# limacv/VideoLoop3D

Measured on AMD Instinct MI355X. Metric: rendered Mpix/s (fwd+bwd) D=32 planes 720p, higher is better.
Workload: dtype f32; 1 GPU; cfg3 stage-2 MPV render fwd+bwd: D=32 planes, T=50 frames, 720x1280, mpv convention, plane stack (D,T,H,W,4) f32 resident in HBM; parallelism=single GPU, variant=0

## Files before the change

videoloop3d_amd/csrc/vl3d_render_bwd_choice.h:

```cpp
#pragma once
#include <stdint.h>
#include "vl3d.h"

namespace vl3d_render_detail {

enum BwdPolicy : int {
    BWD_NONE = 0,
    BWD_AUTO,
    BWD_TILE16,
    BWD_FLAT8,
    BWD_NARROW32,
    BWD_PAIRS32,
    BWD_PAIRS64X12,
};
struct BwdSetting {
    BwdPolicy policy;
    bool gather9;
    bool owner4;
};

inline BwdSetting bwd_setting_of(int entry, int bv, bool tile_ok, bool has_quad_map) {
    BwdSetting s{BWD_NONE, bv == 4, bv != 3 && bv != 4};
    if (entry == VL3D_BWD_ENTRY_ADAM) {
        s.gather9 = s.owner4 = false;
        s.policy = has_quad_map ? (bv == 3 ? BWD_TILE16 : BWD_NARROW32) : BWD_AUTO;
    } else if (bv == 1 || !tile_ok) {
        s.policy = BWD_NONE;
    } else if (entry == VL3D_BWD_ENTRY_MASK) {
        s.policy = (bv == 3 || bv == 4) ? BWD_TILE16 : BWD_FLAT8;
    } else {
        s.policy = bv == 0 ? BWD_AUTO : bv == 2 ? BWD_FLAT8 : bv == 5 ? BWD_NARROW32 : bv == 6 ? BWD_PAIRS32 : bv == 7 ? BWD_PAIRS64X12 : BWD_TILE16;
    }
    return s;
}

enum BwdShape : int { BWD_64X16 = 0, BWD_64X8, BWD_32X16, BWD_64X12, BWD_NSHAPES };
struct BwdRegion { int width, rows; };
constexpr BwdRegion BWD_REGIONS[BWD_NSHAPES] = {{64, 16}, {64, 8}, {32, 16}, {64, 12}};
constexpr int BWD_HALO = 1;
constexpr int bwd_interior_w(int shape) { return BWD_REGIONS[shape].width - 2 * BWD_HALO; }
constexpr int bwd_interior_h(int shape) { return BWD_REGIONS[shape].rows - 2 * BWD_HALO; }
constexpr int bwd_slot_bits(int shape) { return BWD_REGIONS[shape].width * BWD_REGIONS[shape].rows > 512 ? 10 : 9; }

constexpr BwdRegion BWD_SIZING_ONLY_INTERIORS[] = {{60, 12}, {28, 12}};
inline int64_t bwd_max_tiles(int H, int W) {
    auto ntiles = [&](int iw, int ih) { return (int64_t)((W + iw - 1) / iw) * ((H + ih - 1) / ih); };
    int64_t tiles = 0;
    for (int s = 0; s < BWD_NSHAPES; ++s) tiles = ntiles(bwd_interior_w(s), bwd_interior_h(s)) > tiles ? ntiles(bwd_interior_w(s), bwd_interior_h(s)) : tiles;
    for (const BwdRegion &r : BWD_SIZING_ONLY_INTERIORS) tiles = ntiles(r.width, r.rows) > tiles ? ntiles(r.width, r.rows) : tiles;
    return tiles;
}

struct BwdChoice {
    int family;
    BwdShape shape;
    bool reg, mask, adam, cull, f16;
    bool owner4;
};

constexpr int bwd_key(int family, int shape, bool reg, bool mask = false, bool adam = false) {
    return family | shape << 2 | (int)reg << 5 | (int)mask << 6 | (int)adam << 7;
}
inline int bwd_key(const BwdChoice &c) { return bwd_key(c.family, c.shape, c.reg, c.mask, c.adam); }

struct BwdFacts {
    int coord, border, order, ract, aact;
    bool f16;
    int plane_record;
    int T, H, W, Hs, Ws;
    BwdSetting set;
    bool reg, mask, adam, qk, gcu;
};

inline BwdChoice choose_bwd(const BwdFacts &f) {
    const BwdPolicy p = f.set.policy;
    const bool sig = f.ract == VL3D_ACT_SIGMOID && f.aact == VL3D_ACT_SIGMOID;
    const bool shipped = f.coord == VL3D_COORD_AFFINE && f.border == VL3D_BORDER_HARDCUT && f.order == VL3D_ACT_POST && sig && !f.f16;
    const bool shipped9 = shipped && f.plane_record == 9;
    BwdChoice c{VL3D_BWD_TILE, BWD_64X16, false, false, false, false, false, false};
    c.owner4 = f.T == 1 && !f.adam && f.set.owner4;
    if (p == BWD_NONE) { c.family = VL3D_BWD_ATOMICS; c.owner4 = false; return c; }
    if (f.mask && shipped) { c.shape = p == BWD_FLAT8 ? BWD_64X8 : BWD_64X16; c.reg = f.reg; c.mask = true; return c; }
    if (f.adam && shipped9) {
        c.adam = true;
        if (f.qk) { c.shape = p == BWD_TILE16 ? BWD_64X16 : BWD_32X16; c.reg = c.cull = true; return c; }
        c.family = VL3D_BWD_PAIR; c.shape = BWD_32X16; c.reg = f.reg;
        return c;
    }
    if (sig && f.T >= 2 && !f.qk) {
        const bool fits = (int64_t)f.Hs * 100 <= (int64_t)f.H * 107 || (int64_t)f.Ws * 100 <= (int64_t)f.W * 107;
        if ((p == BWD_AUTO || p == BWD_PAIRS32 || p == BWD_PAIRS64X12) && !f.reg && fits) {
            c.family = p == BWD_PAIRS32 ? VL3D_BWD_PAIR : VL3D_BWD_PAIR12;
            c.shape = p == BWD_PAIRS32 ? BWD_32X16 : BWD_64X12;
            c.f16 = f.f16;
            return c;
        }
        if (f.coord != VL3D_COORD_UTILS_MPI && p == BWD_AUTO && f.reg) {
            c.family = VL3D_BWD_PAIR; c.shape = BWD_32X16; c.reg = true; c.f16 = f.f16;
            return c;
        }
    }
    if (shipped9 && (p == BWD_NARROW32 || (p == BWD_AUTO && f.qk && f.gcu))) {
        c.shape = BWD_32X16; c.reg = f.reg || (p == BWD_NARROW32 && f.qk && f.gcu); c.cull = f.qk;
        return c;
    }
    if (shipped9 && !f.reg && !f.qk && (p == BWD_FLAT8 || (p == BWD_AUTO && f.T == 1))) { c.shape = BWD_64X8; return c; }
    c.reg = f.reg || (f.qk && f.gcu); c.cull = f.qk; c.f16 = f.f16;
    return c;
}

}
```

videoloop3d_amd/csrc/vl3d_render_core.h:

```cpp
#pragma once
#include <stddef.h>
#include "vl3d_common.h"
#include "vl3d_bake_rule.h"

#include "vl3d_adam.h"
#include "vl3d_render_bwd_choice.h"

#ifndef VL3D_HS
#define VL3D_HS 9
#define VL3D_HN 9
#endif

namespace vl3d_render_detail {

#ifndef VL3D_PAIR_MIN_WAVES
#define VL3D_PAIR_MIN_WAVES 4
#endif
#ifndef VL3D_FWD2X_MIN_WAVES
#define VL3D_FWD2X_MIN_WAVES 4
#endif

#ifdef VL3D_REG_ABLATE
#define VL3D_REGAB(bit) ((VL3D_REG_ABLATE & (bit)) != 0)
#else
// ... 1388 lines not shown
                }
            continue;
        }
        float2 tc = make_float2(0.f, 0.f);
        float4 gval = make_float4(0.f, 0.f, 0.f, 0.f);
        f4 o = f4{0.f, 0.f, 0.f, 0.f}, pre = o;
        Taps2 tp{};
        float gm = 0.f, msig = 0.f;
        if (inimg) {
            if constexpr (CULL) tp = make_taps2<COORD, BORDER>(h, px, py, a.Hs, a.Ws, a.sx, a.sy, a.ox, a.oy, plane_cull(a, d));
            else tp = make_taps2<COORD, BORDER>(h, px, py, a.Hs, a.Ws, a.sx, a.sy, a.ox, a.oy);
            const char *src = plane;
            if VL3D_ABLATE(a.ablate, 4) {
                src = reinterpret_cast<const char *>(a.stack);
                tp.off &= 0xfff0u;
            }
            typename TapVal<F16, ORDER>::type tv[4];
            load_taps2<F16>(src, tp, st, tv);
            float mt[4];
            if constexpr (MASK) load_mask_taps(mplane, tp.off, st, mt);
            o = shade2<ORDER, RACT, AACT>(tp, tv, &pre);
            if constexpr (MASK) msig = act_fwd<VL3D_ACT_SIGMOID>(mask_blend(mt, tp.w));
        }
        f4 sg = f4{0.f, 0.f, 0.f, 0.f};
        if constexpr (REG) if (reg_on) {
            if ((d >> 2) != wg_idx) {
                wg_idx = d >> 2;
                const uint2 *w = sgp + (size_t)(d >> 2) * sg_plane;
                const uint2 zz = make_uint2(0x55555555u, 0x55555555u);
                wg_own = w[0]; wg_l = w[has_l ? -1 : 0]; wg_u = w[has_u ? -(ptrdiff_t)a.W : 0];
                if (!has_l) wg_l = zz;
                if (!has_u) wg_u = zz;
                if (fl & 12u) wg_p = reinterpret_cast<const uint2 *>(a.reg_patch)[w - reinterpret_cast<const uint2 *>(a.reg_signs)];
            }
            const bool hi = (d & 2) != 0;
            sg = reg_grad32(hi ? wg_own.y : wg_own.x, hi ? wg_l.y : wg_l.x, hi ? wg_u.y : wg_u.x, hi ? wg_p.y : wg_p.x, 16u * (d & 1), fl,
                            f4{gsx_c, gsx_c, gsx_c, gsx_a}, f4{gsy_c, gsy_c, gsy_c, gsy_a});
        }
        if (inimg) {
            const float q = dot3p(Gr, o.x, Gg, o.y, Gb, o.z, gA);
            const float w = o.w * Tr;
            if constexpr (MASK) gm = gL * w * (msig * (1.0f - msig));
            P = fmaf(w, q, P);
            const float om = 1.0f - o.w;
            const float behind = (om > 1e-12f) ? (S - P) * fast_rcp(om) : 0.0f;
            if constexpr (REG) sg.w += fmaf(gN2, o.w, gN1);
            gval = make_float4(fmaf(w, Gr, sg.x), fmaf(w, Gg, sg.y), fmaf(w, Gb, sg.z), fmaf(Tr, q, -behind) + sg.w);
            Tr *= om;
            if constexpr (ORDER == VL3D_ACT_POST)
                gval = make_float4(gval.x * act_bwd<RACT>(pre.x, o.x), gval.y * act_bwd<RACT>(pre.y, o.y),
                                   gval.z * act_bwd<RACT>(pre.z, o.z), gval.w * act_bwd<AACT>(pre.w, o.w));
            tc = make_float2(tp.tx, tp.ty);
            if (!(tp.cov > 0.0f && provider)) gval = make_float4(0.f, 0.f, 0.f, 0.f);
        }
        s_t[buf][tid] = tc;
        s_g[buf][tid] = gval;
        if constexpr (MASK) s_gm[buf][tid] = gm;
        f4 pre_m = f4{0.f, 0.f, 0.f, 0.f}, pre_v = pre_m, pre_p = pre_m;
        if constexpr (ADAM && CULL) {
            const bool mine0 = row < wh && lane < ww && (e0 >> SLOT_BITS) == my_tile && (rec0.x & 3u) == 1u;
            const size_t fb = adam_frame_base(a, d, t), o = mine0 ? (size_t)rec0.y << 4 : 0;
            pre_m = *reinterpret_cast<const f4 *>(reinterpret_cast<const char *>(a.ad.m) + fb + o);
            pre_v = *reinterpret_cast<const f4 *>(reinterpret_cast<const char *>(a.ad.v) + fb + o);
            pre_p = load_texel<false>(plane, mine0 ? (win0 + toff_thread) << 4 : 0u);
            asm volatile("" ::: "memory");
        }
        __syncthreads();
        if VL3D_ABLATE(a.ablate, 1) continue;
        auto gather = [&](unsigned e, int wx, int wy, unsigned tix, uint2 rec = make_uint2(0u, 0u), bool pre = false) {
            if ((e >> SLOT_BITS) != my_tile) return;
            const int lc = (int)(e & SLOT_MASK);
            const f2 tau = f2{(float)(X0 + wx), (float)(Y0 + wy)};
            f4 acc = f4{0.f, 0.f, 0.f, 0.f};
            float accm = 0.f;
            if VL3D_ABLATE(a.ablate, 8) {
            } else if (apart) {
                const f2 c0 = *reinterpret_cast<const f2 *>(&s_t[buf][lc]);
                const int li0 = lc - (tau.x < c0.x ? 1 : 0) - (tau.y < c0.y ? RW : 0);
#pragma unroll
                for (int k = 0; k < 4; ++k) {
                    const int li = li0 + (k >> 1) * RW + (k & 1);
                    const f2 dc = *reinterpret_cast<const f2 *>(&s_t[buf][li]) - tau;
                    const float wgt = tent_weight(dc.x) * tent_weight(dc.y);
                    acc += *reinterpret_cast<const f4 *>(&s_g[buf][li]) * wgt;
                    if constexpr (MASK) accm = fmaf(s_gm[buf][li], wgt, accm);
                }
            } else {
#pragma unroll
            for (int dy = -1; dy <= 1; ++dy)
#pragma unroll
                for (int dx = -1; dx <= 1; ++dx) {
                    const int li = lc + dy * RW + dx;
                    const f2 dc = *reinterpret_cast<const f2 *>(&s_t[buf][li]) - tau;
                    const float wgt = tent_weight(dc.x) * tent_weight(dc.y);
                    if (!a.gather9 && __builtin_amdgcn_ballot_w64(wgt != 0.0f) == 0ull) continue;
                    acc += *reinterpret_cast<const f4 *>(&s_g[buf][li]) * wgt;
                    if constexpr (MASK) accm = fmaf(s_gm[buf][li], wgt, accm);
                }
            }
            if constexpr (ORDER == VL3D_ACT_PRE || ORDER == VL3D_ACT_BAKED) {
                const f4 sv = load_texel<F16>(plane, tix << 4);
                acc = f4{acc.x * act_bwd<RACT>(sv.x, act_fwd<RACT>(sv.x)), acc.y * act_bwd<RACT>(sv.y, act_fwd<RACT>(sv.y)),
                         acc.z * act_bwd<RACT>(sv.z, act_fwd<RACT>(sv.z)), acc.w * act_bwd<AACT>(sv.w, act_fwd<AACT>(sv.w))};
            }
            if constexpr (ADAM) {
                int from;
                if constexpr (CULL) {
                    const unsigned c = rec.x & 3u;
                    if (c == 2) store_grad_texel<false>(gplane, tix << 4, acc);
                    if (c != 1) return;
                    from = (int)(rec.x >> 2);
                    const size_t offp = (size_t)rec.y << 4;
                    if (pre) adam_texel_step_mv(a, adam_frame_base(a, d, t), offp, from, pre_p, acc, pre_m, pre_v);
                    else adam_texel_step(a, adam_frame_base(a, d, t), offp, from, load_texel<false>(plane, tix << 4), acc);
                } else {
                    unsigned off;
                    if (!adam_texel(a, d, X0 + wx, Y0 + wy, from, off)) return;
                    adam_texel_step(a, adam_frame_base(a, d, t), off, from, load_texel<false>(plane, tix << 4), acc);
                }
            } else if (!VL3D_ABLATE(a.ablate, 2)) store_grad_texel<F16>(gplane, tix << 4, acc);
            if constexpr (MASK) __builtin_nontemporal_store(accm, gmplane + tix);
        };
        auto rec_at = [&](unsigned tix) { if constexpr (ADAM && CULL) return rplane[tix]; else return make_uint2(0u, 0u); };
        if (row < wh && lane < ww) gather(e0, lane, row, win0 + toff_thread, rec0, true);
        const int nec = ww - RW;
        if (nec > 0 && nec <= RW) {
            const int sh = nec > 1 ? 32 - __builtin_clz((unsigned)(nec - 1)) : 0, rpw = RW >> sh, rmain = min(wh, ROWS);
            const int c = lane & ((1 << sh) - 1), r = lane >> sh;
            for (int wy0 = row * rpw; wy0 < rmain; wy0 += ROWS * rpw) {
                const int wy = wy0 + r, wx = RW + c;
                if (c < nec && wy < rmain) {
                    const unsigned tix = win0 + (unsigned)(wy * a.Ws + wx);
                    gather(oplane[tix], wx, wy, tix, rec_at(tix));
                }
            }
        } else if (nec > RW) {
            for (int wx = lane + RW; wx < ww && row < wh; wx += RW) {
                const unsigned tix = win0 + (unsigned)(row * a.Ws + wx);
                gather(oplane[tix], wx, row, tix, rec_at(tix));
            }
        }
        for (int wy = row + ROWS; wy < wh; wy += ROWS)
            for (int wx = lane; wx < ww; wx += RW) {
                const unsigned tix = win0 + (unsigned)(wy * a.Ws + wx);
                gather(oplane[tix], wx, wy, tix, rec_at(tix));
            }
    }
}



constexpr int PROWS = 16;

template <int ORDER, int RACT, int AACT, bool F16, bool ADAM = false, int PW = 32, int PR = PROWS>
__device__ __forceinline__ void pair_gather_plane(const RenderArgs &a, const float4 *sg0, const float4 *sg1, const float2 *st, int X0, int Y0,
                                                  int ww, int wh, bool apart, unsigned my_tile, unsigned e0, const unsigned short *oplane,
                                                  const char *plane0, char *gplane0, size_t f1, size_t frame_b, bool has1, int col, int row,
                                                  int d = 0, int t0 = 0) {
    const unsigned win0 = (unsigned)(Y0 * a.Ws + X0);
    auto gather = [&](unsigned e, int wx, int wy, unsigned tix) {
        constexpr int SLOT_BITS = PW == 64 ? 10 : 9;
        if ((e >> SLOT_BITS) != my_tile) return;
        const int lc = (int)(e & ((1u << SLOT_BITS) - 1u));
        const f2 tau = f2{(float)(X0 + wx), (float)(Y0 + wy)};
        f4 acc0 = f4{0.f, 0.f, 0.f, 0.f}, acc1 = acc0;
        if (apart) {
            const f2 c0 = *reinterpret_cast<const f2 *>(&st[lc]);
            const int li0 = lc - (tau.x < c0.x ? 1 : 0) - (tau.y < c0.y ? PW : 0);
#pragma unroll
            for (int k = 0; k < 4; ++k) {
                const int li = li0 + (k >> 1) * PW + (k & 1);
                const f2 dc = *reinterpret_cast<const f2 *>(&st[li]) - tau;
                const float wgt = tent_weight(dc.x) * tent_weight(dc.y);
                acc0 += *reinterpret_cast<const f4 *>(&sg0[li]) * wgt;
                acc1 += *reinterpret_cast<const f4 *>(&sg1[li]) * wgt;
            }
        } else {
#pragma unroll
            for (int dy = -1; dy <= 1; ++dy)
#pragma unroll
                for (int dx = -1; dx <= 1; ++dx) {
                    const int li = lc + dy * PW + dx;
                    const f2 dc = *reinterpret_cast<const f2 *>(&st[li]) - tau;
                    const float wgt = tent_weight(dc.x) * tent_weight(dc.y);
                    if (!a.gather9 && __builtin_amdgcn_ballot_w64(wgt != 0.0f) == 0ull) continue;
                    acc0 += *reinterpret_cast<const f4 *>(&sg0[li]) * wgt;
                    acc1 += *reinterpret_cast<const f4 *>(&sg1[li]) * wgt;
                }
        }
        if constexpr (ORDER == VL3D_ACT_PRE || ORDER == VL3D_ACT_BAKED) {
            const f4 sv0 = load_texel<F16>(plane0, tix << 4), sv1 = load_texel<F16>(plane0 + f1, tix << 4);
            acc0 = f4{acc0.x * act_bwd<RACT>(sv0.x, act_fwd<RACT>(sv0.x)), acc0.y * act_bwd<RACT>(sv0.y, act_fwd<RACT>(sv0.y)),
                      acc0.z * act_bwd<RACT>(sv0.z, act_fwd<RACT>(sv0.z)), acc0.w * act_bwd<AACT>(sv0.w, act_fwd<AACT>(sv0.w))};
            acc1 = f4{acc1.x * act_bwd<RACT>(sv1.x, act_fwd<RACT>(sv1.x)), acc1.y * act_bwd<RACT>(sv1.y, act_fwd<RACT>(sv1.y)),
                      acc1.z * act_bwd<RACT>(sv1.z, act_fwd<RACT>(sv1.z)), acc1.w * act_bwd<AACT>(sv1.w, act_fwd<AACT>(sv1.w))};
        }
        if constexpr (ADAM) {
            static_assert(!F16, "the fused optimiser step: fp32 stacks");
            int from;
            unsigned off;
            if (!adam_texel(a, d, X0 + wx, Y0 + wy, from, off)) return;
            const size_t fbytes = (size_t)a.ad.Hs * a.ad.Ws * 16, fb = ((size_t)d * a.T + t0) * fbytes;
            adam_texel_step(a, fb, off, from, load_texel<false>(plane0, tix << 4), acc0);
            if (has1) adam_texel_step(a, fb + fbytes, off, from, load_texel<false>(plane0 + f1, tix << 4), acc1);
        } else {
            store_grad_texel<F16>(gplane0, tix << 4, acc0);
            if (has1) store_grad_texel<F16>(gplane0 + frame_b, tix << 4, acc1);
        }
    };
    if (row < wh && col < ww) gather(e0, col, row, win0 + (unsigned)(row * a.Ws + col));
    const int nec = ww - PW;
    if (nec > 0) {
        const int necp = min(nec, PW);
        const int sh = necp > 1 ? 32 - __builtin_clz((unsigned)(necp - 1)) : 0, rpg = PW >> sh, rmain = min(wh, PR);
        const int c = col & ((1 << sh) - 1), r = col >> sh;
        for (int wxb = PW; wxb < ww; wxb += (1 << sh))
            for (int wy0 = row * rpg; wy0 < rmain; wy0 += PR * rpg) {
                const int wy = wy0 + r, wx = wxb + c;
                if (c < necp && wx < ww && wy < rmain) {
                    const unsigned tix = win0 + (unsigned)(wy * a.Ws + wx);
                    gather(oplane[tix], wx, wy, tix);
                }
            }
    }
    for (int wy = row + PR; wy < wh; wy += PR)
        for (int wx = col; wx < ww; wx += PW) {
            const unsigned tix = win0 + (unsigned)(wy * a.Ws + wx);
            gather(oplane[tix], wx, wy, tix);
        }
}

#define VL3D_PAIR_GRAD(o, pre, Gr, Gg, Gb, gA, S, P, Tr, gv, ex)                                                               \
    {                                                                                                                          \
        const float q = dot3p(Gr, o.x, Gg, o.y, Gb, o.z, gA);                                                                  \
        const float w = o.w * Tr;                                                                                              \
        P = fmaf(w, q, P);                                                                                                     \
        const float om = 1.0f - o.w;                                                                                           \
        const float behind = (om > 1e-12f) ? (S - P) * fast_rcp(om) : 0.0f;                                                    \
        gv = make_float4(fmaf(w, Gr, ex.x), fmaf(w, Gg, ex.y), fmaf(w, Gb, ex.z), fmaf(Tr, q, -behind) + ex.w);                \
        Tr *= om;                                                                                                              \
        if constexpr (ORDER == VL3D_ACT_POST)                                                                                  \
            gv = make_float4(gv.x * act_bwd<RACT>(pre.x, o.x), gv.y * act_bwd<RACT>(pre.y, o.y),                              \
                             gv.z * act_bwd<RACT>(pre.z, o.z), gv.w * act_bwd<AACT>(pre.w, o.w));                              \
    }

template <int COORD, int BORDER, int ORDER, int RACT, int AACT, bool F16, bool REG = false, bool ADAM = false, int PW = 32>
__global__ __launch_bounds__(PW * PROWS, VL3D_PAIR_MIN_WAVES) void render_bwd_pair_k(RenderArgs a) {
    static_assert(PW == 32 || PW == 64, "region width");
    constexpr int PNT = PW * PROWS;
    if (!reinterpret_cast<const int *>(a.plan)[0]) return;
    __shared__ float4 s_g[2][2][PNT];
    __shared__ float2 s_t[2][PNT];
    const int tid = threadIdx.x, col = tid & (PW - 1), row = tid / PW;
    const int bid = xcd_remap(blockIdx.x, gridDim.x);
    const int tile_x = bid % a.tiles_x, rest = bid / a.tiles_x;
    const int tile_y = rest % a.tiles_y, t0 = (rest / a.tiles_y) * 2;
    const bool has1 = t0 + 1 < a.T;
    const int rx0 = tile_x * (PW - 2) - 1, ry0 = tile_y * (PROWS - 2) - 1;
    const int x = rx0 + col, y = ry0 + row;
    const bool inimg = (x >= 0) && (x < a.W) && (y >= 0) && (y < a.H);
    const float px = (float)(a.col0 + x) + a.pc, py = (float)(a.row0 + y) + a.pc;
    constexpr size_t TEXB = F16 ? 8 : 16;
    const size_t frame_b = (size_t)a.Hs * a.Ws * TEXB;
    const size_t plane_stride_b = (size_t)a.T * frame_b;
    const char *plane0 = reinterpret_cast<const char *>(a.stack) + (size_t)t0 * frame_b;
    char *gplane0 = reinterpret_cast<char *>(a.g_stack) + (size_t)t0 * frame_b;
    const size_t f1 = has1 ? frame_b : 0;
    float Gr0 = 0.f, Gg0 = 0.f, Gb0 = 0.f, gA0 = 0.f, S0 = 0.f, Gr1 = 0.f, Gg1 = 0.f, Gb1 = 0.f, gA1 = 0.f, S1 = 0.f;
    if (inimg) {
        size_t pix = ((size_t)t0 * a.H + y) * a.W + x;
        Gr0 = a.g_rgb[pix * 3 + 0]; Gg0 = a.g_rgb[pix * 3 + 1]; Gb0 = a.g_rgb[pix * 3 + 2];
        gA0 = a.g_alpha ? a.g_alpha[pix] : 0.0f;
        S0 = dot3p(Gr0, a.rgb[pix * 3 + 0], Gg0, a.rgb[pix * 3 + 1], Gb0, a.rgb[pix * 3 + 2], gA0 * a.alpha[pix]);
        if (has1) pix += (size_t)a.H * a.W;
        Gr1 = a.g_rgb[pix * 3 + 0]; Gg1 = a.g_rgb[pix * 3 + 1]; Gb1 = a.g_rgb[pix * 3 + 2];
        gA1 = a.g_alpha ? a.g_alpha[pix] : 0.0f;
        S1 = dot3p(Gr1, a.rgb[pix * 3 + 0], Gg1, a.rgb[pix * 3 + 1], Gb1, a.rgb[pix * 3 + 2], gA1 * a.alpha[pix]);
    }
    float gN10 = 0.f, gN20 = 0.f, gN11 = 0.f, gN21 = 0.f;
    f4 gx = f4{0.f, 0.f, 0.f, 0.f}, gy = gx;
    unsigned fl = 0u;
    const uint2 *sgp = nullptr;
    uint2 go0 = make_uint2(0u, 0u), gl0 = go0, gu0 = go0, gp0 = go0, go1 = go0, gl1 = go0, gu1 = go0, gp1 = go0;
    const bool has_l = inimg && x >= 1, has_u = inimg && y >= 1;
    const bool reg_on = REG && a.g_reg != nullptr;
    const size_t sg_plane = (size_t)a.T * a.H * a.W, sg_f1 = has1 ? (size_t)a.H * a.W : 0;
    if constexpr (REG) {
        if (inimg && a.g_asum) {
            size_t pix = ((size_t)t0 * a.H + y) * a.W + x;
            gN10 = a.g_asum[pix * 2 + 0]; gN20 = 2.0f * a.g_asum[pix * 2 + 1];
            pix += sg_f1;
            gN11 = a.g_asum[pix * 2 + 0]; gN21 = 2.0f * a.g_asum[pix * 2 + 1];
        }
        if (reg_on) {
            gx = f4{a.g_reg[0], a.g_reg[0], a.g_reg[0], a.g_reg[2]}; gy = f4{a.g_reg[1], a.g_reg[1], a.g_reg[1], a.g_reg[3]};
            const int xc = min(max(x, 0), a.W - 1), yc = min(max(y, 0), a.H - 1);
            sgp = reinterpret_cast<const uint2 *>(a.reg_signs) + ((size_t)t0 * a.H + yc) * a.W + xc;
            if (inimg) fl = a.reg_flags[(size_t)y * a.W + x];
        }
    }
    float Tr0 = 1.0f, P0 = 0.0f, Tr1 = 1.0f, P1 = 0.0f;
    const TapStep st = make_tap_step<F16>(a.Hs, a.Ws);
    const unsigned my_tile_id = (unsigned)(tile_y * a.tiles_x + tile_x);
    const unsigned my_tile = (unsigned)((tile_y & (PW == 64 ? 7 : 15)) << 3 | (tile_x & 7));
    const unsigned toff_thread = (unsigned)(row * a.Ws + col);
    const cint_p wrec = (cint_p)a.plan + plan_win_off(a.D) + (size_t)my_tile_id * a.D * 4;
    typedef typename TapVal<F16, ORDER>::type tapv_t;
    for (int d = 0; d < a.D; ++d, plane0 += plane_stride_b, gplane0 += plane_stride_b) {
        float h[VL3D_HN];
        load_uniform(a.homos + VL3D_HS * d, h);
        const int X0 = wrec[4 * d], Y0 = wrec[4 * d + 1], wwh = wrec[4 * d + 2];
        const int ww = wwh & 0xffff, wh = (wwh >> 16) & 0x3fff;
        const bool apart = (wwh & 0x40000000) != 0;
        const int buf = d & 1;
        const unsigned short *oplane = a.owner + (size_t)d * a.Hs * a.Ws;
        const unsigned e0 = oplane[(unsigned)(Y0 * a.Ws + X0) + toff_thread];
        if constexpr (REG) if (reg_on && (d & 3) == 0 && !VL3D_REGAB(16)) {
            const uint2 *w = sgp;
            sgp += sg_plane;
            const ptrdiff_t ol = has_l ? -1 : 0, ou = has_u ? -(ptrdiff_t)a.W : 0;
            const uint2 zz = make_uint2(0x55555555u, 0x55555555u);
            go0 = w[0]; gl0 = w[ol]; gu0 = w[ou];
            go1 = w[sg_f1]; gl1 = w[sg_f1 + ol]; gu1 = w[sg_f1 + ou];
            if (!has_l) { gl0 = zz; gl1 = zz; }
            if (!has_u) { gu0 = zz; gu1 = zz; }
            if (fl & 12u) {
                const uint2 *pw = reinterpret_cast<const uint2 *>(a.reg_patch) + (w - reinterpret_cast<const uint2 *>(a.reg_signs));
                gp0 = pw[0]; gp1 = pw[sg_f1];
            }
        }
        float2 tc = make_float2(0.f, 0.f);
        float4 gv0 = make_float4(0.f, 0.f, 0.f, 0.f), gv1 = gv0;
        if (inimg) {
            const Taps2 tp = make_taps2<COORD, BORDER>(h, px, py, a.Hs, a.Ws, a.sx, a.sy, a.ox, a.oy);
            tapv_t tv0[4], tv1[4];
            load_taps2<F16>(plane0, tp, st, tv0);
            load_taps2<F16>(plane0 + f1, tp, st, tv1);
            f4 pre0, pre1;
            const f4 o0 = shade2<ORDER, RACT, AACT>(tp, tv0, &pre0);
            const f4 o1 = shade2<ORDER, RACT, AACT>(tp, tv1, &pre1);
            f4 ex0 = f4{0.f, 0.f, 0.f, 0.f}, ex1 = ex0;
            if constexpr (REG) {
                if (reg_on && !VL3D_REGAB(8)) {
                    const bool hi = (d & 2) != 0;
                    const unsigned bo = 16u * (d & 1);
                    ex0 = reg_grad32(hi ? go0.y : go0.x, hi ? gl0.y : gl0.x, hi ? gu0.y : gu0.x, hi ? gp0.y : gp0.x, bo, fl, gx, gy);
                    ex1 = reg_grad32(hi ? go1.y : go1.x, hi ? gl1.y : gl1.x, hi ? gu1.y : gu1.x, hi ? gp1.y : gp1.x, bo, fl, gx, gy);
                }
                ex0.w += fmaf(gN20, o0.w, gN10);
                ex1.w += fmaf(gN21, o1.w, gN11);
            }
            VL3D_PAIR_GRAD(o0, pre0, Gr0, Gg0, Gb0, gA0, S0, P0, Tr0, gv0, ex0)
            VL3D_PAIR_GRAD(o1, pre1, Gr1, Gg1, Gb1, gA1, S1, P1, Tr1, gv1, ex1)
            tc = make_float2(tp.tx, tp.ty);
            if (!(tp.cov > 0.0f)) { gv0 = make_float4(0.f, 0.f, 0.f, 0.f); gv1 = gv0; }
        }
        s_t[buf][tid] = tc;
        s_g[buf][0][tid] = gv0;
        s_g[buf][1][tid] = gv1;
        __syncthreads();
        pair_gather_plane<ORDER, RACT, AACT, F16, ADAM, PW>(a, s_g[buf][0], s_g[buf][1], s_t[buf], X0, Y0, ww, wh, apart, my_tile, e0, oplane, plane0,
                                                        gplane0, f1, frame_b, has1, col, row, d, t0);
    }
}

template <int COORD, int BORDER, int ORDER, int RACT, int AACT, bool F16, bool REG = false, bool ADAM = false>
void launch_pair(const RenderArgs &a, hipStream_t s, const BwdChoice &) {
    constexpr int SHAPE = BWD_32X16, PW = BWD_REGIONS[SHAPE].width, RH = BWD_HALO, IW = bwd_interior_w(SHAPE), IH = bwd_interior_h(SHAPE);
    static_assert(PROWS == BWD_REGIONS[SHAPE].rows, "render_bwd_pair_k's rows are not the shape table's");
    RenderArgs b = a;
    b.tiles_x = (a.W + IW - 1) / IW; b.tiles_y = (a.H + IH - 1) / IH;
    const int nwin = b.tiles_x * b.tiles_y * a.D;
    hipLaunchKernelGGL((bwd_windows_k<COORD>), dim3((nwin + 255) / 256), dim3(256), 0, s, b, IW, IH, RH, b.tiles_x, b.tiles_y,
                       reinterpret_cast<int *>(const_cast<float *>(a.plan)) + plan_win_off(a.D));
    hipLaunchKernelGGL(bwd_owner_table_k, dim3((a.Ws + 63) / 64, (a.Hs + 3) / 4, a.D), dim3(256), 0, s, b, IW, IH, RH, b.tiles_x,
                       const_cast<unsigned short *>(a.owner), PW, bwd_slot_bits(SHAPE));
    hipLaunchKernelGGL((render_bwd_pair_k<COORD, BORDER, ORDER, RACT, AACT, F16, REG, ADAM, PW>),
                       dim3((unsigned)(b.tiles_x * b.tiles_y * ((a.T + 1) / 2))), dim3(PW * PROWS), 0, s, b);
}

constexpr int P12W = 64, P12ROWS = 12;
template <int COORD, int BORDER, int ORDER, int RACT, int AACT, bool F16>
__global__ __launch_bounds__(P12W * P12ROWS, 6) void render_bwd_pair12_k(RenderArgs a) {
    constexpr int PW = P12W, PR = P12ROWS, PNT = PW * PR;
    if (!reinterpret_cast<const int *>(a.plan)[0]) return;
    __shared__ float4 s_g[2][2][PNT];
    __shared__ float2 s_t[2][PNT];
    const int tid = threadIdx.x, col = tid & (PW - 1), row = tid / PW;
    const int bid = xcd_remap(blockIdx.x, gridDim.x);
    const int tile_x = bid % a.tiles_x, rest = bid / a.tiles_x;
    const int tile_y = rest % a.tiles_y, t0 = (rest / a.tiles_y) * 2;
    const bool has1 = t0 + 1 < a.T;
    const int rx0 = tile_x * (PW - 2) - 1, ry0 = tile_y * (PR - 2) - 1;
    const int x = rx0 + col, y = ry0 + row;
    const bool inimg = (x >= 0) && (x < a.W) && (y >= 0) && (y < a.H);
    const float px = (float)(a.col0 + x) + a.pc, py = (float)(a.row0 + y) + a.pc;
    constexpr size_t TEXB = F16 ? 8 : 16;
    const size_t frame_b = (size_t)a.Hs * a.Ws * TEXB;
    const size_t plane_stride_b = (size_t)a.T * frame_b;
    const char *plane0 = reinterpret_cast<const char *>(a.stack) + (size_t)t0 * frame_b;
    char *gplane0 = reinterpret_cast<char *>(a.g_stack) + (size_t)t0 * frame_b;
    const size_t f1 = has1 ? frame_b : 0;
    float Gr0 = 0.f, Gg0 = 0.f, Gb0 = 0.f, gA0 = 0.f, S0 = 0.f, Gr1 = 0.f, Gg1 = 0.f, Gb1 = 0.f, gA1 = 0.f, S1 = 0.f;
    if (inimg) {
        size_t pix = ((size_t)t0 * a.H + y) * a.W + x;
        Gr0 = a.g_rgb[pix * 3 + 0]; Gg0 = a.g_rgb[pix * 3 + 1]; Gb0 = a.g_rgb[pix * 3 + 2];
        gA0 = a.g_alpha ? a.g_alpha[pix] : 0.0f;
        S0 = dot3p(Gr0, a.rgb[pix * 3 + 0], Gg0, a.rgb[pix * 3 + 1], Gb0, a.rgb[pix * 3 + 2], gA0 * a.alpha[pix]);
        if (has1) pix += (size_t)a.H * a.W;
        Gr1 = a.g_rgb[pix * 3 + 0]; Gg1 = a.g_rgb[pix * 3 + 1]; Gb1 = a.g_rgb[pix * 3 + 2];
        gA1 = a.g_alpha ? a.g_alpha[pix] : 0.0f;
        S1 = dot3p(Gr1, a.rgb[pix * 3 + 0], Gg1, a.rgb[pix * 3 + 1], Gb1, a.rgb[pix * 3 + 2], gA1 * a.alpha[pix]);
    }
    float Tr0 = 1.0f, P0 = 0.0f, Tr1 = 1.0f, P1 = 0.0f;
    const TapStep st = make_tap_step<F16>(a.Hs, a.Ws);
    const unsigned my_tile_id = (unsigned)(tile_y * a.tiles_x + tile_x);
    const unsigned my_tile = (unsigned)((tile_y & 7) << 3 | (tile_x & 7));
    const unsigned toff_thread = (unsigned)(row * a.Ws + col);
    const cint_p wrec = (cint_p)a.plan + plan_win_off(a.D) + (size_t)my_tile_id * a.D * 4;
    typedef typename TapVal<F16, ORDER>::type tapv_t;
    const f4 ex = f4{0.f, 0.f, 0.f, 0.f};
    for (int d = 0; d < a.D; ++d, plane0 += plane_stride_b, gplane0 += plane_stride_b) {
        float h[VL3D_HN];
        load_uniform(a.homos + VL3D_HS * d, h);
        const int X0 = wrec[4 * d], Y0 = wrec[4 * d + 1], wwh = wrec[4 * d + 2];
        const int ww = wwh & 0xffff, wh = (wwh >> 16) & 0x3fff;
        const bool apart = (wwh & 0x40000000) != 0;
        const int buf = d & 1;
        const unsigned short *oplane = a.owner + (size_t)d * a.Hs * a.Ws;
        const unsigned e0 = oplane[(unsigned)(Y0 * a.Ws + X0) + toff_thread];
        float2 tc = make_float2(0.f, 0.f);
        float4 gv0 = make_float4(0.f, 0.f, 0.f, 0.f), gv1 = gv0;
        if (inimg) {
            const Taps2 tp = make_taps2<COORD, BORDER>(h, px, py, a.Hs, a.Ws, a.sx, a.sy, a.ox, a.oy);
            tapv_t tv0[4], tv1[4];
            load_taps2<F16>(plane0, tp, st, tv0);
            load_taps2<F16>(plane0 + f1, tp, st, tv1);
            f4 pre0, pre1;
            const f4 o0 = shade2<ORDER, RACT, AACT>(tp, tv0, &pre0);
            const f4 o1 = shade2<ORDER, RACT, AACT>(tp, tv1, &pre1);
            VL3D_PAIR_GRAD(o0, pre0, Gr0, Gg0, Gb0, gA0, S0, P0, Tr0, gv0, ex)
            VL3D_PAIR_GRAD(o1, pre1, Gr1, Gg1, Gb1, gA1, S1, P1, Tr1, gv1, ex)
            tc = make_float2(tp.tx, tp.ty);
            if (!(tp.cov > 0.0f)) { gv0 = make_float4(0.f, 0.f, 0.f, 0.f); gv1 = gv0; }
        }
        s_t[buf][tid] = tc;
        s_g[buf][0][tid] = gv0;
        s_g[buf][1][tid] = gv1;
        __syncthreads();
        pair_gather_plane<ORDER, RACT, AACT, F16, false, PW, PR>(a, s_g[buf][0], s_g[buf][1], s_t[buf], X0, Y0, ww, wh, apart, my_tile, e0, oplane, plane0,
                                                                 gplane0, f1, frame_b, has1, col, row, d, t0);
    }
}

#undef VL3D_PAIR_GRAD

template <int COORD, int BORDER, int ORDER, int RACT, int AACT, bool F16>
void launch_pair12(const RenderArgs &a, hipStream_t s, const BwdChoice &) {
    constexpr int SHAPE = BWD_64X12, RH = BWD_HALO, IW = bwd_interior_w(SHAPE), IH = bwd_interior_h(SHAPE);
    static_assert(P12W == BWD_REGIONS[SHAPE].width && P12ROWS == BWD_REGIONS[SHAPE].rows, "render_bwd_pair12_k's region is not the shape table's");
    RenderArgs b = a;
    b.tiles_x = (a.W + IW - 1) / IW; b.tiles_y = (a.H + IH - 1) / IH;
    const int nwin = b.tiles_x * b.tiles_y * a.D;
    hipLaunchKernelGGL((bwd_windows_k<COORD>), dim3((nwin + 255) / 256), dim3(256), 0, s, b, IW, IH, RH, b.tiles_x, b.tiles_y,
                       reinterpret_cast<int *>(const_cast<float *>(a.plan)) + plan_win_off(a.D));
    hipLaunchKernelGGL(bwd_owner_table_k, dim3((a.Ws + 63) / 64, (a.Hs + 3) / 4, a.D), dim3(256), 0, s, b, IW, IH, RH, b.tiles_x,
                       const_cast<unsigned short *>(a.owner), P12W, bwd_slot_bits(SHAPE));
    hipLaunchKernelGGL((render_bwd_pair12_k<COORD, BORDER, ORDER, RACT, AACT, F16>),
                       dim3((unsigned)(b.tiles_x * b.tiles_y * ((a.T + 1) / 2))), dim3(P12W * P12ROWS), 0, s, b);
}

template <int COORD, int BORDER, int ORDER, int RACT, int AACT, bool F16, bool MASK = false>
__global__ __launch_bounds__(512) void render_fwd_reg_k(RenderArgs a, int tiles_x, int tiles_y) {
    constexpr int FW = 64, FH = 8, NT = FW * FH;
    __shared__ float4 s_o[2][NT];
    __shared__ float red[4][FH];
    const int b = xcd_remap(blockIdx.x, gridDim.x);
    const int tile_x = b % tiles_x, rest = b / tiles_x;
    const int tile_y = rest % tiles_y, t = rest / tiles_y;
    const int tid = threadIdx.x, lane = tid & 63, row = tid >> 6;
    const int x = tile_x * (FW - 1) + lane, y = tile_y * (FH - 1) + row;
    const bool inimg = (x < a.W) && (y < a.H);
    const bool owner = inimg && lane < FW - 1 && row < FH - 1;
    const unsigned fl = owner ? a.reg_flags[(size_t)y * a.W + x] : 0u;
    const bool own_r = owner && x + 1 < a.W && !(fl & 1u), own_d = owner && y + 1 < a.H && !(fl & 2u);
    const size_t sg_plane = (size_t)a.T * a.H * a.W;
    uint2 *sgq = reinterpret_cast<uint2 *>(a.reg_signs) + ((size_t)t * a.H + min(y, a.H - 1)) * a.W + min(x, a.W - 1);
    unsigned sg_lo = 0u, sg_hi = 0u;
    const float px = (float)(a.col0 + min(x, a.W - 1)) + a.pc, py = (float)(a.row0 + min(y, a.H - 1)) + a.pc;
    const size_t frame_b = (size_t)a.Hs * a.Ws * (F16 ? 8 : 16), plane_stride_b = (size_t)a.T * frame_b;
    const char *plane = reinterpret_cast<const char *>(a.stack) + (size_t)t * frame_b;
    float Tr = 1.0f, cr = 0.f, cg = 0.f, cb = 0.f, A = 0.f, n1 = 0.f, n2 = 0.f;
    float sxc = 0.f, syc = 0.f, sxa = 0.f, sya = 0.f;
    const TapStep st = make_tap_step<F16>(a.Hs, a.Ws);
    typedef typename TapVal<F16, ORDER>::type tapv_t;
    tapv_t vA[4], vB[4];
    static_assert(!(MASK && F16), "the loop-mask channel: fp32 stage-1 stacks");
    float mA[4] = {0.f, 0.f, 0.f, 0.f}, mB[4] = {0.f, 0.f, 0.f, 0.f}, lab = 0.f;
    const float *mplane = MASK ? a.mask + (size_t)t * a.Hs * a.Ws : nullptr;
    const size_t mplane_stride = (size_t)a.T * a.Hs * a.Ws;
#define VL3D_PLANE(T_, V_, BUF_, S_, M_)                                                                  \
    {                                                                                                     \
        const f4 o = shade2<ORDER, RACT, AACT>(T_, V_);                                                   \
        const f4 ol = inimg ? o * T_.cov : f4{0.f, 0.f, 0.f, 0.f};                                        \
        if (!VL3D_REGAB(4)) s_o[BUF_][tid] = make_float4(ol.x, ol.y, ol.z, ol.w);                         \
        const float w = o.w * Tr;                                                                         \
        cr += w * o.x; cg += w * o.y; cb += w * o.z; A += w;                                              \
        n1 += o.w; n2 = fmaf(o.w, o.w, n2);                                                               \
        Tr *= (1.0f - o.w);                                                                               \
        if constexpr (MASK) lab = fmaf(w, act_fwd<VL3D_ACT_SIGMOID>(mask_blend(M_, T_.w)), lab);          \
        if (!VL3D_REGAB(4)) __syncthreads();                                                              \
        int code = (int)REG_ZERO;                                                                         \
        if (own_r && !VL3D_REGAB(2)) {                                                                    \
            const float4 r = s_o[BUF_][tid + 1];                                                          \
            const f4 df = ol - f4{r.x, r.y, r.z, r.w};                                                    \
            sxc += fabsf(df.x) + fabsf(df.y) + fabsf(df.z);                                               \
            sxa += fabsf(df.w);                                                                           \
            if (!VL3D_REGAB(1)) code += reg_signs4(df);                                                   \
        }                                                                                                 \
        if (own_d && !VL3D_REGAB(2)) {                                                                    \
            const float4 r = s_o[BUF_][tid + FW];                                                         \
            const f4 df = ol - f4{r.x, r.y, r.z, r.w};                                                    \
            syc += fabsf(df.x) + fabsf(df.y) + fabsf(df.z);                                               \
            sya += fabsf(df.w);                                                                           \
            if (!VL3D_REGAB(1)) code += reg_signs4(df) << 8;                                              \
        }                                                                                                 \
        if (VL3D_REGAB(1)) { }                                                                            \
        else if (S_ == 0) sg_lo = (unsigned)code;                                                         \
        else if (S_ == 1) sg_lo |= (unsigned)code << 16;                                                  \
        else if (S_ == 2) sg_hi = (unsigned)code;                                                         \
        else {                                                                                            \
            sg_hi |= (unsigned)code << 16;                                                                \
            if (owner) *sgq = make_uint2(sg_lo, sg_hi);                                                   \
            sgq += sg_plane;                                                                              \
        }                                                                                                 \
    }
    const QuadCull noq = QuadCull{nullptr, 0, 0, 0.f, 0.f, 0.f, 0.f, 0};
    Taps2 tA = make_taps2<COORD, BORDER>(a.homos, px, py, a.Hs, a.Ws, a.sx, a.sy, a.ox, a.oy, noq, UvNoise{a.uv_seed, 0}), tB = tA;
    load_taps2<F16>(plane, tA, st, vA);
    if constexpr (MASK) load_mask_taps(mplane, tA.off, st, mA);
#define VL3D_FETCH(T_, V_, DN_, M_)                                                                       \
    {                                                                                                     \
        const int dn = min(DN_, a.D - 1);                                                                 \
        float h[VL3D_HN];                                                                                 \
        load_uniform(a.homos + VL3D_HS * dn, h);                                                          \
        T_ = make_taps2<COORD, BORDER>(h, px, py, a.Hs, a.Ws, a.sx, a.sy, a.ox, a.oy, noq, UvNoise{a.uv_seed, dn});  \
        load_taps2<F16>(plane + (size_t)dn * plane_stride_b, T_, st, V_);                                 \
        if constexpr (MASK) load_mask_taps(mplane + (size_t)dn * mplane_stride, T_.off, st, M_);          \
        asm volatile("" ::: "memory");                                                                    \
    }
    int d = 0;
    for (;; d += 4) {
        VL3D_FETCH(tB, vB, d + 1, mB)
        VL3D_PLANE(tA, vA, 0, 0, mA)
        if (d + 1 >= a.D) break;
        VL3D_FETCH(tA, vA, d + 2, mA)
        VL3D_PLANE(tB, vB, 1, 1, mB)
        if (d + 2 >= a.D) break;
        VL3D_FETCH(tB, vB, d + 3, mB)
        VL3D_PLANE(tA, vA, 0, 2, mA)
        if (d + 3 >= a.D) break;
        VL3D_FETCH(tA, vA, d + 4, mA)
        VL3D_PLANE(tB, vB, 1, 3, mB)
        if (d + 4 >= a.D) break;
    }
    if ((a.D & 3) && owner) *sgq = make_uint2(sg_lo, (a.D & 3) == 3 ? sg_hi : 0u);
#undef VL3D_FETCH
#undef VL3D_PLANE
    if (owner) {
        const size_t pix = ((size_t)t * a.H + y) * a.W + x;
        a.rgb[pix * 3 + 0] = cr; a.rgb[pix * 3 + 1] = cg; a.rgb[pix * 3 + 2] = cb;
        a.alpha[pix] = A;
        if (a.asum) { a.asum[pix * 2 + 0] = n1; a.asum[pix * 2 + 1] = n2; }
        if constexpr (MASK) a.label[pix] = lab;
    }
    float v[4] = {sxc, syc, sxa, sya};
#pragma unroll
    for (int k = 0; k < 4; ++k) {
#pragma unroll
        for (int off = 32; off > 0; off >>= 1) v[k] += __shfl_down(v[k], off, 64);
        if (lane == 0) red[k][row] = v[k];
    }
    __syncthreads();
    if (tid < 4) {
        double sum = 0.0;
        for (int r = 0; r < FH; ++r) sum += (double)red[tid][r];
        atomicAdd(a.reg_sums + tid, sum);
    }
}

template <int COORD, int BORDER, int ORDER, int RACT, int AACT, int SHAPE, bool REG, bool F16 = false, bool MASK = false, bool ADAM = false>
void launch_tile(const RenderArgs &a, hipStream_t s, const BwdChoice &c) {
    constexpr int RWT = BWD_REGIONS[SHAPE].width, ROWS = BWD_REGIONS[SHAPE].rows, RH = BWD_HALO, IW = bwd_interior_w(SHAPE), IH = bwd_interior_h(SHAPE);
    constexpr int SLOT_BITS = bwd_slot_bits(SHAPE);
    RenderArgs b = a;
    b.tiles_x = (a.W + IW - 1) / IW; b.tiles_y = (a.H + IH - 1) / IH;
    const int nwin = b.tiles_x * b.tiles_y * a.D;
    hipLaunchKernelGGL((bwd_windows_k<COORD>), dim3((nwin + 255) / 256), dim3(256), 0, s, b, IW, IH, RH, b.tiles_x, b.tiles_y,
                       reinterpret_cast<int *>(const_cast<float *>(a.plan)) + plan_win_off(a.D));
    if (c.owner4)
        hipLaunchKernelGGL(bwd_owner_table4_k, dim3(((a.Ws + 3) / 4 + 63) / 64, (a.Hs + 3) / 4, a.D), dim3(256), 0, s, b, IW, IH, RH,
                           const_cast<unsigned short *>(a.owner), RWT, SLOT_BITS);
    else
        hipLaunchKernelGGL(bwd_owner_table_k, dim3((a.Ws + 63) / 64, (a.Hs + 3) / 4, a.D), dim3(256), 0, s, b, IW, IH, RH, b.tiles_x,
                           const_cast<unsigned short *>(a.owner), RWT, SLOT_BITS);
    const dim3 grid((unsigned)(b.tiles_x * b.tiles_y * a.T)), block(RWT * ROWS);
    if constexpr (ADAM) {
        hipLaunchKernelGGL((render_bwd_tile_k<COORD, BORDER, ORDER, RACT, AACT, ROWS, true, false, true, false, true, RWT>), grid, block, 0, s, b);
    } else if constexpr (MASK) {
        hipLaunchKernelGGL((render_bwd_tile_k<COORD, BORDER, ORDER, RACT, AACT, ROWS, REG, F16, false, true, false, RWT>), grid, block, 0, s, b);
    } else if (c.cull)
        hipLaunchKernelGGL((render_bwd_tile_k<COORD, BORDER, ORDER, RACT, AACT, ROWS, REG, F16, true, false, false, RWT>), grid, block, 0, s, b);
    else
        hipLaunchKernelGGL((render_bwd_tile_k<COORD, BORDER, ORDER, RACT, AACT, ROWS, REG, F16, false, false, false, RWT>), grid, block, 0, s, b);
}

using BwdLauncher = void (*)(const RenderArgs &, hipStream_t, const BwdChoice &);

inline BwdFacts bwd_facts_of(const RenderArgs &a, int coord, int border, int order, int ract, int aact, bool f16, int plane_record) {
    BwdFacts f{};
    f.coord = coord; f.border = border; f.order = order; f.ract = ract; f.aact = aact; f.f16 = f16; f.plane_record = plane_record;
    f.T = a.T; f.H = a.H; f.W = a.W; f.Hs = a.Hs; f.Ws = a.Ws;
// ... 116 lines not shown
```

Measured before the change: 2652 Mpix/s.

## Add ownerless pair12 backward that recomputes texel owners instead of owner table

Adds an ownerless variant of the 64x12 pair backward kernel. It skips building and reading the per-texel owner table and instead recomputes each texel's owning pixel from the inverse homography inside the gather. Texels whose owner falls near or outside the image border are zeroed by a separate small kernel. The f32 auto path turns this on by default. It trades the owner table writes and reads for extra per-texel arithmetic and a border-zeroing pass, and depends on the recomputed owner matching the table semantics exactly.

```diff
diff --git a/videoloop3d_amd/csrc/vl3d_render_bwd_choice.h b/videoloop3d_amd/csrc/vl3d_render_bwd_choice.h
--- a/videoloop3d_amd/csrc/vl3d_render_bwd_choice.h
+++ b/videoloop3d_amd/csrc/vl3d_render_bwd_choice.h
@@ -12,6 +12,7 @@
     BWD_NARROW32,
     BWD_PAIRS32,
     BWD_PAIRS64X12,
+    BWD_PAIRS64X12O,
 };
 struct BwdSetting {
     BwdPolicy policy;
@@ -29,7 +30,7 @@
     } else if (entry == VL3D_BWD_ENTRY_MASK) {
         s.policy = (bv == 3 || bv == 4) ? BWD_TILE16 : BWD_FLAT8;
     } else {
-        s.policy = bv == 0 ? BWD_AUTO : bv == 2 ? BWD_FLAT8 : bv == 5 ? BWD_NARROW32 : bv == 6 ? BWD_PAIRS32 : bv == 7 ? BWD_PAIRS64X12 : BWD_TILE16;
+        s.policy = bv == 0 ? BWD_AUTO : bv == 2 ? BWD_FLAT8 : bv == 5 ? BWD_NARROW32 : bv == 6 ? BWD_PAIRS32 : bv == 7 ? BWD_PAIRS64X12 : bv == 8 ? BWD_PAIRS64X12O : BWD_TILE16;
     }
     return s;
 }
@@ -51,11 +52,14 @@
     return tiles;
 }
 
+constexpr bool BWD_PAIR12_AUTO_OWNERLESS_F32 = true, BWD_PAIR12_AUTO_OWNERLESS_F16 = false;
+
 struct BwdChoice {
     int family;
     BwdShape shape;
     bool reg, mask, adam, cull, f16;
     bool owner4;
+    bool ownerless;
 };
 
 constexpr int bwd_key(int family, int shape, bool reg, bool mask = false, bool adam = false) {
@@ -73,11 +77,13 @@
 };
 
 inline BwdChoice choose_bwd(const BwdFacts &f) {
-    const BwdPolicy p = f.set.policy;
     const bool sig = f.ract == VL3D_ACT_SIGMOID && f.aact == VL3D_ACT_SIGMOID;
+    const bool fits = (int64_t)f.Hs * 100 <= (int64_t)f.H * 107 || (int64_t)f.Ws * 100 <= (int64_t)f.W * 107;
+    const bool plain_pairs = sig && f.T >= 2 && !f.qk && !f.adam && !f.mask && !f.reg && fits;
+    const BwdPolicy p = f.set.policy == BWD_PAIRS64X12O && !plain_pairs ? BWD_AUTO : f.set.policy;
     const bool shipped = f.coord == VL3D_COORD_AFFINE && f.border == VL3D_BORDER_HARDCUT && f.order == VL3D_ACT_POST && sig && !f.f16;
     const bool shipped9 = shipped && f.plane_record == 9;
-    BwdChoice c{VL3D_BWD_TILE, BWD_64X16, false, false, false, false, false, false};
+    BwdChoice c{VL3D_BWD_TILE, BWD_64X16, false, false, false, false, false, false, false};
     c.owner4 = f.T == 1 && !f.adam && f.set.owner4;
     if (p == BWD_NONE) { c.family = VL3D_BWD_ATOMICS; c.owner4 = false; return c; }
     if (f.mask && shipped) { c.shape = p == BWD_FLAT8 ? BWD_64X8 : BWD_64X16; c.reg = f.reg; c.mask = true; return c; }
@@ -88,11 +94,12 @@
         return c;
     }
     if (sig && f.T >= 2 && !f.qk) {
-        const bool fits = (int64_t)f.Hs * 100 <= (int64_t)f.H * 107 || (int64_t)f.Ws * 100 <= (int64_t)f.W * 107;
-        if ((p == BWD_AUTO || p == BWD_PAIRS32 || p == BWD_PAIRS64X12) && !f.reg && fits) {
+        if ((p == BWD_AUTO || p == BWD_PAIRS32 || p == BWD_PAIRS64X12 || p == BWD_PAIRS64X12O) && !f.reg && fits) {
             c.family = p == BWD_PAIRS32 ? VL3D_BWD_PAIR : VL3D_BWD_PAIR12;
             c.shape = p == BWD_PAIRS32 ? BWD_32X16 : BWD_64X12;
             c.f16 = f.f16;
+            c.ownerless = p == BWD_PAIRS64X12O ||
+                          (p == BWD_AUTO && f.coord != VL3D_COORD_UTILS_MPI && (f.f16 ? BWD_PAIR12_AUTO_OWNERLESS_F16 : BWD_PAIR12_AUTO_OWNERLESS_F32));
             return c;
         }
         if (f.coord != VL3D_COORD_UTILS_MPI && p == BWD_AUTO && f.reg) {
diff --git a/videoloop3d_amd/csrc/vl3d_render_core.h b/videoloop3d_amd/csrc/vl3d_render_core.h
--- a/videoloop3d_amd/csrc/vl3d_render_core.h
+++ b/videoloop3d_amd/csrc/vl3d_render_core.h
@@ -1564,15 +1564,31 @@
 
 constexpr int PROWS = 16;
 
-template <int ORDER, int RACT, int AACT, bool F16, bool ADAM = false, int PW = 32, int PR = PROWS>
+template <int ORDER, int RACT, int AACT, bool F16, bool ADAM = false, int PW = 32, int PR = PROWS, bool OWNERLESS = false>
 __device__ __forceinline__ void pair_gather_plane(const RenderArgs &a, const float4 *sg0, const float4 *sg1, const float2 *st, int X0, int Y0,
                                                   int ww, int wh, bool apart, unsigned my_tile, unsigned e0, const unsigned short *oplane,
                                                   const char *plane0, char *gplane0, size_t f1, size_t frame_b, bool has1, int col, int row,
-                                                  int d = 0, int t0 = 0) {
+                                                  int d = 0, int t0 = 0, const float *hi = nullptr, int ix0 = 0, int ix1 = 0, int iy0 = 0,
+                                                  int iy1 = 0) {
     const unsigned win0 = (unsigned)(Y0 * a.Ws + X0);
+    [[maybe_unused]] float wmax = 0.0f, hmax = 0.0f;
+    if constexpr (OWNERLESS) {
+        wmax = __int_as_float(__builtin_amdgcn_readfirstlane(__float_as_int((float)(a.W - 1))));
+        hmax = __int_as_float(__builtin_amdgcn_readfirstlane(__float_as_int((float)(a.H - 1))));
+    }
     auto gather = [&](unsigned e, int wx, int wy, unsigned tix) {
         constexpr int SLOT_BITS = PW == 64 ? 10 : 9;
-        if ((e >> SLOT_BITS) != my_tile) return;
+        if constexpr (OWNERLESS) {
+            int c0 = a.col0, r0 = a.row0;
+            asm volatile("" : "+s"(c0), "+s"(r0));
+            float qx, qy;
+            owner_pixel(hi, (float)(X0 + wx), (float)(Y0 + wy), a.pc, c0, r0, qx, qy);
+            const int rx = (int)fminf(fmaxf(rintf(qx), 0.0f), wmax), ry = (int)fminf(fmaxf(rintf(qy), 0.0f), hmax);
+            if (rx < ix0 || rx > ix1 || ry < iy0 || ry > iy1) return;
+            e = (unsigned)((ry - iy0 + BWD_HALO) * PW + (rx - ix0 + BWD_HALO));
+        } else {
+            if ((e >> SLOT_BITS) != my_tile) return;
+        }
         const int lc = (int)(e & ((1u << SLOT_BITS) - 1u));
         const f2 tau = f2{(float)(X0 + wx), (float)(Y0 + wy)};
         f4 acc0 = f4{0.f, 0.f, 0.f, 0.f}, acc1 = acc0;
@@ -1631,14 +1647,16 @@
                 const int wy = wy0 + r, wx = wxb + c;
                 if (c < necp && wx < ww && wy < rmain) {
                     const unsigned tix = win0 + (unsigned)(wy * a.Ws + wx);
-                    gather(oplane[tix], wx, wy, tix);
+                    if constexpr (OWNERLESS) gather(0u, wx, wy, tix);
+                    else gather(oplane[tix], wx, wy, tix);
                 }
             }
     }
     for (int wy = row + PR; wy < wh; wy += PR)
         for (int wx = col; wx < ww; wx += PW) {
             const unsigned tix = win0 + (unsigned)(wy * a.Ws + wx);
-            gather(oplane[tix], wx, wy, tix);
+            if constexpr (OWNERLESS) gather(0u, wx, wy, tix);
+            else gather(oplane[tix], wx, wy, tix);
         }
 }
 
@@ -1865,10 +1883,101 @@
     }
 }
 
+template <int COORD, int BORDER, int ORDER, int RACT, int AACT, bool F16>
+__global__ __launch_bounds__(P12W * P12ROWS, 6) void render_bwd_pair12o_k(RenderArgs a) {
+    constexpr int PW = P12W, PR = P12ROWS, PNT = PW * PR;
+    if (!reinterpret_cast<const int *>(a.plan)[0]) return;
+    __shared__ float4 s_g[2][2][PNT];
+    __shared__ float2 s_t[2][PNT];
+    const int tid = threadIdx.x, col = tid & (PW - 1), row = tid / PW;
+    const int bid = xcd_remap(blockIdx.x, gridDim.x);
+    const int tile_x = bid % a.tiles_x, rest = bid / a.tiles_x;
+    const int tile_y = rest % a.tiles_y, t0 = (rest / a.tiles_y) * 2;
+    const bool has1 = t0 + 1 < a.T;
+    const int rx0 = tile_x * (PW - 2) - 1, ry0 = tile_y * (PR - 2) - 1;
+    const int x = rx0 + col, y = ry0 + row;
+    const bool inimg = (x >= 0) && (x < a.W) && (y >= 0) && (y < a.H);
+    const float px = (float)(a.col0 + x) + a.pc, py = (float)(a.row0 + y) + a.pc;
+    const int ix0 = tile_x * (PW - 2), ix1 = min(ix0 + (PW - 2) - 1, a.W - 1), iy0 = tile_y * (PR - 2), iy1 = min(iy0 + (PR - 2) - 1, a.H - 1);
+    constexpr size_t TEXB = F16 ? 8 : 16;
+    const size_t frame_b = (size_t)a.Hs * a.Ws * TEXB;
+    const size_t plane_stride_b = (size_t)a.T * frame_b;
+    const char *plane0 = reinterpret_cast<const char *>(a.stack) + (size_t)t0 * frame_b;
+    char *gplane0 = reinterpret_cast<char *>(a.g_stack) + (size_t)t0 * frame_b;
+    const size_t f1 = has1 ? frame_b : 0;
+    float Gr0 = 0.f, Gg0 = 0.f, Gb0 = 0.f, gA0 = 0.f, S0 = 0.f, Gr1 = 0.f, Gg1 = 0.f, Gb1 = 0.f, gA1 = 0.f, S1 = 0.f;
+    if (inimg) {
+        size_t pix = ((size_t)t0 * a.H + y) * a.W + x;
+        Gr0 = a.g_rgb[pix * 3 + 0]; Gg0 = a.g_rgb[pix * 3 + 1]; Gb0 = a.g_rgb[pix * 3 + 2];
+        gA0 = a.g_alpha ? a.g_alpha[pix] : 0.0f;
+        S0 = dot3p(Gr0, a.rgb[pix * 3 + 0], Gg0, a.rgb[pix * 3 + 1], Gb0, a.rgb[pix * 3 + 2], gA0 * a.alpha[pix]);
+        if (has1) pix += (size_t)a.H * a.W;
+        Gr1 = a.g_rgb[pix * 3 + 0]; Gg1 = a.g_rgb[pix * 3 + 1]; Gb1 = a.g_rgb[pix * 3 + 2];
+        gA1 = a.g_alpha ? a.g_alpha[pix] : 0.0f;
+        S1 = dot3p(Gr1, a.rgb[pix * 3 + 0], Gg1, a.rgb[pix * 3 + 1], Gb1, a.rgb[pix * 3 + 2], gA1 * a.alpha[pix]);
+    }
+    float Tr0 = 1.0f, P0 = 0.0f, Tr1 = 1.0f, P1 = 0.0f;
+    const TapStep st = make_tap_step<F16>(a.Hs, a.Ws);
+    const unsigned my_tile_id = (unsigned)(tile_y * a.tiles_x + tile_x);
+    const cint_p wrec = (cint_p)a.plan + plan_win_off(a.D) + (size_t)my_tile_id * a.D * 4;
+    typedef typename TapVal<F16, ORDER>::type tapv_t;
+    const f4 ex = f4{0.f, 0.f, 0.f, 0.f};
+    for (int d = 0; d < a.D; ++d, plane0 += plane_stride_b, gplane0 += plane_stride_b) {
+        float h[VL3D_HN], hi[9];
+        load_uniform(a.homos + VL3D_HS * d, h);
+        load_uniform(a.plan + PLAN_HDR + PLAN_REC * d, hi);
+        const int X0 = wrec[4 * d], Y0 = wrec[4 * d + 1], wwh = wrec[4 * d + 2];
+        const int ww = wwh & 0xffff, wh = (wwh >> 16) & 0x3fff;
+        const bool apart = (wwh & 0x40000000) != 0;
+        const int buf = d & 1;
+        float2 tc = make_float2(0.f, 0.f);
+        float4 gv0 = make_float4(0.f, 0.f, 0.f, 0.f), gv1 = gv0;
+        if (inimg) {
+            const Taps2 tp = make_taps2<COORD, BORDER>(h, px, py, a.Hs, a.Ws, a.sx, a.sy, a.ox, a.oy);
+            tapv_t tv0[4], tv1[4];
+            load_taps2<F16>(plane0, tp, st, tv0);
+            load_taps2<F16>(plane0 + f1, tp, st, tv1);
+            f4 pre0, pre1;
+            const f4 o0 = shade2<ORDER, RACT, AACT>(tp, tv0, &pre0);
+            const f4 o1 = shade2<ORDER, RACT, AACT>(tp, tv1, &pre1);
+            VL3D_PAIR_GRAD(o0, pre0, Gr0, Gg0, Gb0, gA0, S0, P0, Tr0, gv0, ex)
+            VL3D_PAIR_GRAD(o1, pre1, Gr1, Gg1, Gb1, gA1, S1, P1, Tr1, gv1, ex)
+            tc = make_float2(tp.tx, tp.ty);
+            if (!(tp.cov > 0.0f)) { gv0 = make_float4(0.f, 0.f, 0.f, 0.f); gv1 = gv0; }
+        }
+        s_t[buf][tid] = tc;
+        s_g[buf][0][tid] = gv0;
+        s_g[buf][1][tid] = gv1;
+        __syncthreads();
+        pair_gather_plane<ORDER, RACT, AACT, F16, false, PW, PR, true>(a, s_g[buf][0], s_g[buf][1], s_t[buf], X0, Y0, ww, wh, apart, 0u, 0u, nullptr,
+                                                                       plane0, gplane0, f1, frame_b, has1, col, row, d, t0, hi, ix0, ix1, iy0, iy1);
+    }
+}
+
 #undef VL3D_PAIR_GRAD
 
+__global__ __launch_bounds__(256) void bwd_zero_unowned_k(RenderArgs a) {
+    if (!reinterpret_cast<const int *>(a.plan)[0]) return;
+    const int x = blockIdx.x * 64 + (threadIdx.x & 63);
+    const int y = blockIdx.y * 4 + (threadIdx.x >> 6);
+    const int d = blockIdx.z;
+    if (x >= a.Ws || y >= a.Hs) return;
+    float qx, qy;
+    owner_pixel(a.plan + PLAN_HDR + PLAN_REC * d, (float)x, (float)y, a.pc, a.col0, a.row0, qx, qy);
+    const bool safe = (qx > 0.5f) && (qx < (float)a.W - 1.5f) && (qy > 0.5f) && (qy < (float)a.H - 1.5f);
+    if (safe) return;
+    const size_t frame = (size_t)a.Hs * a.Ws;
+    if (a.g_f16) {
+        float2 *g = reinterpret_cast<float2 *>(a.g_stack) + (size_t)d * a.T * frame + (size_t)y * a.Ws + x;
+        for (int t = 0; t < a.T; ++t, g += frame) *g = make_float2(0.f, 0.f);
+    } else {
+        float4 *g = reinterpret_cast<float4 *>(a.g_stack) + (size_t)d * a.T * frame + (size_t)y * a.Ws + x;
+        for (int t = 0; t < a.T; ++t, g += frame) *g = make_float4(0.f, 0.f, 0.f, 0.f);
+    }
+}
+
 template <int COORD, int BORDER, int ORDER, int RACT, int AACT, bool F16>
-void launch_pair12(const RenderArgs &a, hipStream_t s, const BwdChoice &) {
+void launch_pair12(const RenderArgs &a, hipStream_t s, const BwdChoice &c) {
     constexpr int SHAPE = BWD_64X12, RH = BWD_HALO, IW = bwd_interior_w(SHAPE), IH = bwd_interior_h(SHAPE);
     static_assert(P12W == BWD_REGIONS[SHAPE].width && P12ROWS == BWD_REGIONS[SHAPE].rows, "render_bwd_pair12_k's region is not the shape table's");
     RenderArgs b = a;
@@ -1876,10 +1985,15 @@
     const int nwin = b.tiles_x * b.tiles_y * a.D;
     hipLaunchKernelGGL((bwd_windows_k<COORD>), dim3((nwin + 255) / 256), dim3(256), 0, s, b, IW, IH, RH, b.tiles_x, b.tiles_y,
                        reinterpret_cast<int *>(const_cast<float *>(a.plan)) + plan_win_off(a.D));
+    const dim3 grid((unsigned)(b.tiles_x * b.tiles_y * ((a.T + 1) / 2))), block(P12W * P12ROWS);
+    if (c.ownerless) {
+        hipLaunchKernelGGL(bwd_zero_unowned_k, dim3((a.Ws + 63) / 64, (a.Hs + 3) / 4, a.D), dim3(256), 0, s, b);
+        hipLaunchKernelGGL((render_bwd_pair12o_k<COORD, BORDER, ORDER, RACT, AACT, F16>), grid, block, 0, s, b);
+        return;
+    }
     hipLaunchKernelGGL(bwd_owner_table_k, dim3((a.Ws + 63) / 64, (a.Hs + 3) / 4, a.D), dim3(256), 0, s, b, IW, IH, RH, b.tiles_x,
                        const_cast<unsigned short *>(a.owner), P12W, bwd_slot_bits(SHAPE));
-    hipLaunchKernelGGL((render_bwd_pair12_k<COORD, BORDER, ORDER, RACT, AACT, F16>),
-                       dim3((unsigned)(b.tiles_x * b.tiles_y * ((a.T + 1) / 2))), dim3(P12W * P12ROWS), 0, s, b);
+    hipLaunchKernelGGL((render_bwd_pair12_k<COORD, BORDER, ORDER, RACT, AACT, F16>), grid, block, 0, s, b);
 }
 
 template <int COORD, int BORDER, int ORDER, int RACT, int AACT, bool F16, bool MASK = false>
```

Result: faster. 2740 Mpix/s (median of 6 runs) (+3.3%).
